# Jiang-Muyun/PointNet12

Hardware: AMD Instinct MI355X
Metric: points/sec fwd+bwd, PointNet2 SemSeg B=16x4096 pts (higher is better)
Workload: dtype f32 (wide-layer products: exact bf16x3 operand splits, 6 bf16 MFMAs per fp32 product, fp32 accumulate)

## Files before the change

### include/pn2.h

```cpp
#ifndef PN2_H
#define PN2_H

#include <stdint.h>

#ifdef __cplusplus
extern "C" {
#endif

#define PN2_ABI_VERSION 15

#define PN2_STAT_REPLICAS 8
#define PN2_DWX_REPLICAS 32

#define PN2_OK 0
#define PN2_OK_SPLIT 1
#define PN2_EINVAL (-1)
#define PN2_ELAUNCH (-2)
#define PN2_EUNSUPPORTED (-3)

typedef void *pn2_stream_t;

typedef struct pn2_bn_lazy {
    const double *stats;
    const float *gamma, *beta;
    float eps, momentum;
    float *running_mean, *running_var;
    int64_t *num_batches_tracked;
    float *affine;
    int64_t count;
    int C;
} pn2_bn_lazy;

typedef struct pn2_bn_coef_lazy {
    const double *red;
    const float *gamma;
    const float *affine;
    float *coef;
    float *dgamma, *dbeta;
    int accumulate;
    int64_t count;
    int C;
} pn2_bn_coef_lazy;

int pn2_version(void);
const char *pn2_error_string(int code);
const char *pn2_last_kernel(void);
void pn2_clear_last_kernel(void);

int pn2_set_option(const char *name, int value);
int pn2_get_option(const char *name, int *value);
const char *pn2_option_name(int index);


int64_t pn2_fps_workspace_bytes(int B, int N, int npoint);
int pn2_fps(const float *xyz, int B, int N, const int64_t *start, int npoint, int64_t *out_idx,
            void *work, pn2_stream_t stream);

int pn2_ball_query(const float *xyz, const float *new_xyz, int B, int N, int S, float r2, int nsample,
                   int64_t *out_idx, pn2_stream_t stream);
int64_t pn2_ball_query_workspace_bytes(int B, int N, int S);
int pn2_ball_query_ws(const float *xyz, const float *new_xyz, int B, int N, int S, float r2, int nsample, int64_t *out_idx,
                      void *work, pn2_stream_t stream);

int pn2_square_distance(const float *src, const float *dst, int B, int S, int N, float *out, pn2_stream_t stream);

// ... 108 lines not shown
int pn2_bwd_res_supported(int64_t P, int C_out, int C_in, int Kpool, int masked);
int pn2_conv1x1_bwd(const float *dZ, int ldz, const float *dZp, int ldo, const int32_t *arg, int Kpool,
                    const float *Y, int ldy, const float *coef, const float *W, int ldw, const float *prev_Y,
                    int ld_prev, const float *prev_affine, float *dXout, int ldxo, double *prev_red, float *dW,
                    int lddw, int64_t P, int C_out, int C_in, const pn2_bn_coef_lazy *coef_lazy, pn2_stream_t stream);

typedef struct {
    const float *W;
    const float *bias;
    int K, N, ldw;
} pn2_eval_layer;
int pn2_fused_eval(const float *X, int ldx, const float *xyz, const float *points, const float *new_xyz,
                   const int64_t *idx, int B, int N, int S, int Knb, int D, int xyz_first,
                   const pn2_eval_layer *layers, int L, int pool, float *out, int ldo, pn2_stream_t stream);

int pn2_invert_index(const int64_t *idx, int B, int M, int T, int32_t *members, int32_t *owners, int32_t *scratch,
                     pn2_stream_t stream);
int pn2_three_interp_bwd_seg(const float *grad_out, int ld, int col0, const int32_t *members, const int32_t *owners,
                             const float *weight, int B, int N, int S, int D, float *grad_points2, pn2_stream_t stream);
int pn2_group_affine_bwd_seg(const float *dZ, int ldz, const float *Y, int ldy, const float *coef, const float *xyz,
                             const float *new_xyz, const int32_t *members, const int32_t *owners, int B, int N, int S,
                             int K, int C, float *G, int ldg, float *dWx, int ldwx, float *dwx_scratch,
                             const pn2_bn_coef_lazy *coef_lazy, pn2_stream_t stream);

int64_t pn2_nll_loss_workspace_bytes(int64_t R);
int pn2_nll_loss_fwd(const float *logp, int ld, const int64_t *target, const float *weight, int64_t R, int C,
                     int64_t ignore_index, void *workspace, float *loss, float *denom, pn2_stream_t stream);
int pn2_nll_loss_bwd(const int64_t *target, const float *weight, int64_t R, int C, int64_t ignore_index,
                     const float *grad_loss, const float *denom, float *dlogp, int ld, pn2_stream_t stream);
int64_t pn2_cross_entropy_workspace_bytes(int64_t R);
int pn2_cross_entropy_fwd(const float *x, int ld, int64_t inner, const int64_t *target, const float *weight, int64_t R, int C,
                          int64_t ignore_index, double label_smoothing, int reduction, void *workspace, float *logsum, float *loss,
                          float *denom, pn2_stream_t stream);
int pn2_cross_entropy_bwd(const float *x, int ld, int64_t inner, const int64_t *target, const float *weight, const float *logsum,
                          int64_t R, int C, int64_t ignore_index, double label_smoothing, int reduction, const float *grad_out,
                          const float *denom, float *dx, pn2_stream_t stream);
int pn2_log_softmax_fwd(const float *x, int ldx, int64_t R, int C, float *out, int ldo, pn2_stream_t stream);
int pn2_log_softmax_bwd(const float *grad_out, int ldg, const float *out, int ldo, int64_t R, int C, float *grad_x, int ldgx,
                        pn2_stream_t stream);

int pn2_adam_step(float *param, float *grad, float *exp_avg, float *exp_avg_sq, int64_t n, double lr, double beta1,
                  double beta2, double eps, double weight_decay, int64_t step, const float *lr_dev, int64_t *step_dev,
                  int zero_grad, pn2_stream_t stream);
int pn2_sgd_step(float *param, float *grad, float *momentum_buf, int64_t n, double lr, double momentum, double dampening,
                 double weight_decay, int nesterov, int maximize, int64_t step, const float *lr_dev, int64_t *step_dev,
                 int zero_grad, pn2_stream_t stream);
// ... 124 lines not shown
```

### pointnet12_amd/_lib.py

```python
import ctypes
import os
import subprocess

_HERE = os.path.dirname(os.path.abspath(__file__))
LIB_PATH = os.environ.get("PN2_LIB_PATH") or os.path.join(_HERE, "libpn2_hip.so")
CSRC = os.path.join(_HERE, "csrc")

_vp, _i, _i64, _f, _d = ctypes.c_void_p, ctypes.c_int, ctypes.c_int64, ctypes.c_float, ctypes.c_double

SIGNATURES = {
    "pn2_version": (_i, []),
    "pn2_error_string": (ctypes.c_char_p, [_i]),
    "pn2_last_kernel": (ctypes.c_char_p, []),
    "pn2_clear_last_kernel": (None, []),
    "pn2_set_option": (_i, [ctypes.c_char_p, _i]),
    "pn2_get_option": (_i, [ctypes.c_char_p, _vp]),
    "pn2_option_name": (ctypes.c_char_p, [_i]),
    "pn2_fps_workspace_bytes": (_i64, [_i, _i, _i]),
    "pn2_fps": (_i, [_vp, _i, _i, _vp, _i, _vp, _vp, _vp]),
    "pn2_ball_query": (_i, [_vp, _vp, _i, _i, _i, _f, _i, _vp, _vp]),
    "pn2_ball_query_workspace_bytes": (_i64, [_i, _i, _i]),
    "pn2_ball_query_ws": (_i, [_vp, _vp, _i, _i, _i, _f, _i, _vp, _vp, _vp]),
    "pn2_square_distance": (_i, [_vp, _vp, _i, _i, _i, _vp, _vp]),
    "pn2_three_nn": (_i, [_vp, _vp, _i, _i, _i, _vp, _vp, _vp, _vp]),
# ... 22 lines not shown
    "pn2_conv1x1_wgrad": (_i, [_vp, _i, _vp, _i, _vp, _i, _vp, _i, _vp, _vp, _i, _vp, _vp, _i, _vp,
                               _i64, _i, _i, _vp, _vp]),
    "pn2_conv1x1_wgrad_workspace_bytes": (_i64, [_i64, _i, _i, _i]),
    "pn2_conv1x1_wgrad_ws": (_i, [_vp, _i, _vp, _i, _vp, _i, _vp, _i, _vp, _vp, _i, _vp, _vp, _i, _vp,
                                  _i64, _i, _i, _vp, _vp, _vp]),
    "pn2_conv1x1_wgrad_cf_scratch_bytes": (_i64, []),
    "pn2_conv1x1_wgrad_cf": (_i, [_vp, _i, _vp, _vp, _i, _vp, _i, _vp, _vp, _vp, _i, _i64, _i, _i, _vp, _vp]),
    "pn2_conv1x1_bwd_pair": (_i, [_vp, _i, _vp, _i, _vp, _i, _vp, _i, _vp, _vp, _i, _vp, _i, _vp, _vp, _i, _vp, _vp, _i, _vp, _vp, _i,
                                  _i64, _i, _i, _vp, _vp]),
    "pn2_res_supported": (_i, [_i64, _i, _i]),
    "pn2_bwd_res_supported": (_i, [_i64, _i, _i, _i, _i]),
    "pn2_conv1x1_bwd": (_i, [_vp, _i, _vp, _i, _vp, _i, _vp, _i, _vp, _vp, _i, _vp, _i, _vp, _vp, _i, _vp, _vp, _i,
                             _i64, _i, _i, _vp, _vp]),
    "pn2_conv1x1_bwd_cf_supported": (_i, [_i64, _i, _i, _i]),
    "pn2_conv1x1_bwd_cf_scratch_bytes": (_i64, [_i, _i]),
    "pn2_conv1x1_bwd_cf": (_i, [_vp, _i, _vp, _i, _vp, _vp, _i, _vp, _vp, _i, _vp, _vp, _i, _vp, _vp, _i, _i64, _i, _i, _vp, _vp, _vp]),
    "pn2_conv1x1_bwd_first_supported": (_i, [_i64, _i, _i, _i]),
    "pn2_conv1x1_bwd_first": (_i, [_vp, _i, _vp, _i, _vp, _vp, _i, _vp, _i, _vp, _vp, _vp, _i, _vp, _i, _i, _vp, _i64, _i, _i, _vp, _vp]),
    "pn2_fused_eval": (_i, [_vp, _i, _vp, _vp, _vp, _vp, _i, _i, _i, _i, _i, _i, _vp, _i, _i, _vp, _i, _vp]),
    "pn2_invert_index": (_i, [_vp, _i, _i, _i, _vp, _vp, _vp, _vp]),
    "pn2_three_interp_bwd_seg": (_i, [_vp, _i, _i, _vp, _vp, _vp, _i, _i, _i, _i, _vp, _vp]),
    "pn2_group_affine_bwd_seg": (_i, [_vp, _i, _vp, _i, _vp, _vp, _vp, _vp, _vp, _i, _i, _i, _i, _i, _vp, _i, _vp, _i,
                                         _vp, _vp, _vp]),
    "pn2_nll_loss_workspace_bytes": (_i64, [_i64]),
    "pn2_nll_loss_fwd": (_i, [_vp, _i, _vp, _vp, _i64, _i, _i64, _vp, _vp, _vp, _vp]),
    "pn2_nll_loss_bwd": (_i, [_vp, _vp, _i64, _i, _i64, _vp, _vp, _vp, _i, _vp]),
    "pn2_cross_entropy_workspace_bytes": (_i64, [_i64]),
    "pn2_cross_entropy_fwd": (_i, [_vp, _i, _i64, _vp, _vp, _i64, _i, _i64, _d, _i, _vp, _vp, _vp, _vp, _vp]),
    "pn2_cross_entropy_bwd": (_i, [_vp, _i, _i64, _vp, _vp, _vp, _i64, _i, _i64, _d, _i, _vp, _vp, _vp, _vp]),
    "pn2_log_softmax_fwd": (_i, [_vp, _i, _i64, _i, _vp, _i, _vp]),
    "pn2_log_softmax_bwd": (_i, [_vp, _i, _vp, _i, _i64, _i, _vp, _i, _vp]),
    "pn2_adam_step": (_i, [_vp, _vp, _vp, _vp, _i64, _d, _d, _d, _d, _d, _i64, _vp, _vp, _i, _vp]),
    "pn2_sgd_step": (_i, [_vp, _vp, _vp, _i64, _d, _d, _d, _d, _i, _i, _i64, _vp, _vp, _i, _vp]),
    "pn2_prepare_clouds": (_i, [_vp, _vp, _vp, _vp, _vp, _vp, _vp, _i, _i, _vp, _vp, _vp, _vp]),
    "pn2_prepare_shapes": (_i, [_vp, _i, _vp, _vp, _vp, _vp, _vp, _i, _vp, _vp, _i, _i, _vp, _vp, _vp, _vp]),
    "pn2_point_transform": (_i, [_vp, _i, _vp, _i, _i, _i, _vp, _i, _vp]),
    "pn2_point_transform_workspace_bytes": (_i64, [_i, _i, _i]),
    "pn2_point_transform_bwd": (_i, [_vp, _i, _vp, _i, _vp, _i, _i, _i, _vp, _i, _vp, _vp, _vp]),
    "pn2_bn_max": (_i, [_vp, _i, _vp, _i64, _i, _i, _vp, _i, _vp, _vp]),
    "pn2_pool_bwd_reduce_noact": (_i, [_vp, _i, _vp, _i, _vp, _i, _vp, _i64, _i, _i, _vp, _vp, _vp]),
    "pn2_conv1x1_fwd_gbias": (_i, [_vp, _i, _vp, _i, _vp, _vp, _i, _i64, _vp, _i, _i64, _i, _i, _vp, _vp]),
    "pn2_group_colsum_workspace_bytes": (_i64, [_i64, _i64, _i]),
    "pn2_group_colsum": (_i, [_vp, _i, _vp, _i, _vp, _i64, _i64, _i, _vp, _i, _vp, _vp]),
    "pn2_conv1x1_fwd_multi": (_i, [_vp, _i, _vp, _i, _vp, _vp, _i, _i64, _vp, _i, _i64, _i, _vp, _vp]),
    "pn2_conv1x1_wgrad_multi": (_i, [_vp, _i, _vp, _i, _vp, _vp, _i, _vp, _i, _vp, _i64, _i, _vp]),
    "pn2_conv1x1_dgrad_multi": (_i, [_vp, _i, _vp, _i, _vp, _vp, _i, _vp, _vp, _vp, _i, _i64, _i, _vp]),
# ... 35 lines not shown
CHANNELS_RGB, CHANNELS_BGR = 0, 1
IMAGE_RGB, IMAGE_HSV = 0, 1
IMAGE_ERR_ROWS = 1
KNN_MAX_K = 32
KNN_ERR_LABEL, KNN_ERR_DST = 1, 2
VOXEL_TILE = 1024
VOXEL_MAX_ROWS = 1 << 29
VOXEL_ERR_RANGE, VOXEL_ERR_ROWS = 1, 2
SEGMENT_MAX_COLS = 16
SEGMENT_ERR_RANGE, SEGMENT_ERR_NONFINITE = 4, 8
CLUSTER_ERR_INDEX, CLUSTER_ERR_CELL, CLUSTER_ERR_CAP, CLUSTER_ERR_ROWS = 16, 32, 64, 128


class BnLazy(ctypes.Structure):
    _fields_ = [("stats", _vp), ("gamma", _vp), ("beta", _vp), ("eps", _f), ("momentum", _f), ("running_mean", _vp),
                ("running_var", _vp), ("num_batches_tracked", _vp), ("affine", _vp), ("count", _i64), ("C", _i)]


class BnCoefLazy(ctypes.Structure):
    _fields_ = [("red", _vp), ("gamma", _vp), ("affine", _vp), ("coef", _vp), ("dgamma", _vp), ("dbeta", _vp),
                ("accumulate", _i), ("count", _i64), ("C", _i)]


class EvalLayer(ctypes.Structure):
    _fields_ = [("W", _vp), ("bias", _vp), ("K", _i), ("N", _i), ("ldw", _i)]


class Src(ctypes.Structure):
    _fields_ = [("X", _vp), ("ldx", _i), ("K", _i), ("affine", _vp), ("relu", _i)]


def src_table(entries):
    return (Src * len(entries))(*[Src(x, ldx, k, aff, relu) for x, ldx, k, aff, relu in entries])


class Pn2Error(RuntimeError):
    pass


def build(force=False):
    if force:
        subprocess.check_call(["make", "-C", CSRC, "-s", "clean"])
    subprocess.check_call(["make", "-C", CSRC, "-s", "-j4"])
    return LIB_PATH


# ... 113 lines not shown
```

### pointnet12_amd/csrc/grouped.hip

```cpp
#include "pn2_common.h"
#include "bn_affine.h"

namespace {

using f32x16 = __attribute__((ext_vector_type(16))) float;

__global__ __launch_bounds__(256) void group_affine_fwd_kernel(const float *__restrict__ Zf, int ldz,
                                                               const float *__restrict__ xyz,
                                                               const float *__restrict__ new_xyz,
                                                               const int64_t *__restrict__ idx,
                                                               const float *__restrict__ Wx, int ldwx, int N, int S,
                                                               int K, int C, int64_t P, float *__restrict__ Y, int ldy,
                                                               double *__restrict__ stats) {
    __shared__ double red[256 * 8];
    const int CG = (C + 3) >> 2;
    const int RPB = 256 / CG;
    const int t = threadIdx.x, cg = t % CG, r = t / CG;
    const bool live = r < RPB;
    const int c = cg * 4;
    float wx[4][3];
#pragma unroll
    for (int e = 0; e < 4; ++e)
#pragma unroll
        for (int a = 0; a < 3; ++a) wx[e][a] = (live && c + e < C) ? Wx[(c + e) * ldwx + a] : 0.f;
    float s0[4] = {0.f, 0.f, 0.f, 0.f}, s1[4] = {0.f, 0.f, 0.f, 0.f};
    double st[8] = {0, 0, 0, 0, 0, 0, 0, 0};
    int since = 0;
    if (live) {
        const int64_t stride = (int64_t)gridDim.x * RPB;
        for (int64_t p0 = (int64_t)blockIdx.x * RPB + r; p0 < P; p0 += 4 * stride) {
            int64_t j[4], g[4], b[4];
#pragma unroll
            for (int u = 0; u < 4; ++u) {
                const int64_t p = p0 + u * stride;
                const bool v = p < P;
                g[u] = v ? p / K : 0;
                b[u] = g[u] / S;
                j[u] = v ? idx[p] : 0;
            }
            float4 z[4];
            float d[4][3];
#pragma unroll
            for (int u = 0; u < 4; ++u) {
                const float *q = xyz + (b[u] * N + j[u]) * 3, *ctr = new_xyz + g[u] * 3;
                d[u][0] = q[0] - ctr[0]; d[u][1] = q[1] - ctr[1]; d[u][2] = q[2] - ctr[2];
                z[u] = *reinterpret_cast<const float4 *>(Zf + (b[u] * N + j[u]) * ldz + c);
            }
#pragma unroll
            for (int u = 0; u < 4; ++u) {
                const int64_t p = p0 + u * stride;
                if (p >= P) break;
                float y[4] = {z[u].x, z[u].y, z[u].z, z[u].w};
#pragma unroll
                for (int e = 0; e < 4; ++e) {
                    y[e] = __builtin_fmaf(wx[e][0], d[u][0], y[e]);
                    y[e] = __builtin_fmaf(wx[e][1], d[u][1], y[e]);
                    y[e] = __builtin_fmaf(wx[e][2], d[u][2], y[e]);
                    if (c + e >= C) y[e] = 0.f;
                    s0[e] += y[e];
                    s1[e] = __builtin_fmaf(y[e], y[e], s1[e]);
                }
                *reinterpret_cast<float4 *>(Y + p * ldy + c) = make_float4(y[0], y[1], y[2], y[3]);
                if (++since == 64) {
#pragma unroll
                    for (int e = 0; e < 4; ++e) {
                        st[e] += (double)s0[e]; st[4 + e] += (double)s1[e];
                        s0[e] = 0.f; s1[e] = 0.f;
                    }
                    since = 0;
                }
            }
        }
#pragma unroll
        for (int e = 0; e < 4; ++e) { st[e] += (double)s0[e]; st[4 + e] += (double)s1[e]; }
    }
    if (stats == nullptr) return;
#pragma unroll
    for (int e = 0; e < 8; ++e) red[t * 8 + e] = st[e];
    __syncthreads();
    for (int ch = t; ch < C; ch += 256) {
        const int g4 = ch >> 2, e = ch & 3;
        double a0 = 0.0, a1 = 0.0;
        for (int rr = 0; rr < RPB; ++rr) {
            a0 += red[(rr * CG + g4) * 8 + e];
            a1 += red[(rr * CG + g4) * 8 + 4 + e];
// ... 244 lines not shown
                       int K, int D, int xyz_first, const float *W, int ldw, const float *bias, float *X, int ldx, float *Y, int ldy,
                       int C_out, double *stats, pn2_stream_t stream) {
    PN2_CHECK_ARG(xyz && W && bias && X && Y && B > 0 && N > 0 && S > 0 && K > 0 && D >= 0 && (D == 0 || points) && (idx || K == N));
    PN2_CHECK_ARG(ldw >= 3 + D && ldx % 4 == 0 && ldx >= ((3 + D + 3) & ~3) && ldy % 4 == 0 && ldy >= C_out);
    const int64_t P = (int64_t)B * S * K;
    if (3 + D > 12 || D > 9 || D < 1 || !idx || !new_xyz || ldx > 12 || !(C_out == 32 || C_out == 64) || P % 64 != 0 || P >= (1LL << 31))
        return PN2_EUNSUPPORTED;
    const int64_t slabs = P / 64;
    int64_t grid = pn2_cdiv(slabs, 4);
    const int64_t cap = (int64_t)pn2_num_cus() * 2;
    if (grid > cap) grid = cap;
    if (C_out == 64)
        hipLaunchKernelGGL(group_conv_fwd_kernel<64>, dim3((unsigned)grid), dim3(256), 0, pn2_s(stream), xyz, points, new_xyz, idx, N, S, K,
                           D, xyz_first, W, ldw, bias, X, ldx, Y, ldy, slabs, stats);
    else
        hipLaunchKernelGGL(group_conv_fwd_kernel<32>, dim3((unsigned)grid), dim3(256), 0, pn2_s(stream), xyz, points, new_xyz, idx, N, S, K,
                           D, xyz_first, W, ldw, bias, X, ldx, Y, ldy, slabs, stats);
    return pn2_launch_status();
}

int pn2_group_affine_fwd(const float *Zf, int ldz, const float *xyz, const float *new_xyz, const int64_t *idx,
                         const float *Wx, int ldwx, int B, int N, int S, int K, int C, float *Y, int ldy, double *stats,
                         pn2_stream_t stream) {
    PN2_CHECK_ARG(Zf && xyz && new_xyz && idx && Wx && Y && B > 0 && N > 0 && S > 0 && K > 0 && C > 0 && C <= 1024 &&
                  ldwx >= 3);
    PN2_CHECK_ARG(ldz % 4 == 0 && ldy % 4 == 0 && ldz >= ((C + 3) & ~3) && ldy >= ((C + 3) & ~3));
    const int64_t P = (int64_t)B * S * K;
    const int rpb = 256 / ((C + 3) >> 2);
    int64_t blocks = pn2_cdiv(P, (int64_t)rpb * 8);
    if (blocks > 1024) blocks = 1024;
    hipLaunchKernelGGL(group_affine_fwd_kernel, dim3((unsigned)blocks), dim3(256), 0, pn2_s(stream), Zf, ldz, xyz, new_xyz, idx,
                       Wx, ldwx, N, S, K, C, P, Y, ldy, stats);
    return pn2_launch_status();
}

int pn2_group_affine_bwd(const float *dZ, int ldz, const float *Y, int ldy, const float *coef, const float *xyz,
                         const float *new_xyz, const int64_t *idx, int B, int N, int S, int K, int C, float *G, int ldg,
                         float *dWx, int ldwx, pn2_stream_t stream) {
    PN2_CHECK_ARG(dZ && Y && coef && xyz && new_xyz && idx && G && dWx && B > 0 && N > 0 && S > 0 && K > 0 && C > 0 &&
                  C <= 1024);
    PN2_CHECK_ARG(ldz % 4 == 0 && ldy % 4 == 0 && ldg % 4 == 0 && ldwx >= 3);
    const int64_t P = (int64_t)B * S * K;
    const int rpb = C < 256 ? 256 / C : 1;
    int64_t blocks = pn2_cdiv(P, (int64_t)rpb * 16);
    if (blocks > 768) blocks = 768;
    hipLaunchKernelGGL(group_affine_bwd_kernel, dim3((unsigned)blocks), dim3(256), 0, pn2_s(stream), dZ, ldz, Y, ldy, coef,
                       (C + 3) & ~3, xyz, new_xyz, idx, N, S, K, C, P, G, ldg, dWx, ldwx);
    return pn2_launch_status();
}
// ... 3 lines not shown
```

### pointnet12_amd/csrc/scatter.hip

```cpp
#include "pn2_common.h"
#include "bn_affine.h"
#include <stdlib.h>

namespace {

__device__ __forceinline__ float4 ld4(const float *p) { return *reinterpret_cast<const float4 *>(p); }

__global__ __launch_bounds__(256) void invert_count_kernel(const int64_t *__restrict__ idx, int M, int T,
                                                           int *__restrict__ counts) {
    const int b = blockIdx.y;
    const int m = blockIdx.x * 256 + threadIdx.x;
    if (m >= M) return;
    const int64_t v = idx[(int64_t)b * M + m];
    if (v >= 0 && v < T) atomicAdd(counts + (int64_t)b * T + v, 1);
}

__global__ __launch_bounds__(1024) void invert_scan_kernel(int *__restrict__ counts, int T, int *__restrict__ offsets) {
    __shared__ int wsum[16];
    __shared__ int carry_s;
    const int b = blockIdx.x, t = threadIdx.x, lane = t & 63, wave = t >> 6;
    int *cnt = counts + (int64_t)b * T;
    int *off = offsets + (int64_t)b * (T + 1);
    if (t == 0) carry_s = 0;
    __syncthreads();
// ... 166 lines not shown
                }
            }
#pragma unroll
            for (int u = 0; u < 4; ++u) {
                if (m[u] < 0) continue;
                if (tg[u] != cur) {
                    if (cur >= 0) {
                        row_flush(grad_points2 + (b * S + cur) * D, c, D, acc, !(first && head_shared));
                        first = false;
                    }
                    acc = make_float4(0.f, 0.f, 0.f, 0.f);
                    cur = tg[u];
                }
                float wu = wt[u];
                PN2_OPAQUE1(wu);
                acc.x = __builtin_fmaf(g[u].x, wu, acc.x); acc.y = __builtin_fmaf(g[u].y, wu, acc.y);
                acc.z = __builtin_fmaf(g[u].z, wu, acc.z); acc.w = __builtin_fmaf(g[u].w, wu, acc.w);
            }
        }
        if (cur >= 0) row_flush(grad_points2 + (b * S + cur) * D, c, D, acc, !(first && head_shared) && cur != tail_next);
    }
}

__global__ __launch_bounds__(256) void group_affine_bwd_seg_kernel(const float *__restrict__ dZ, int ldz,
                                                                   const float *__restrict__ Y, int ldy,
                                                                   const float *coef, int ldc,
                                                                   const float *__restrict__ xyz,
                                                                   const float *__restrict__ new_xyz,
                                                                   const int *__restrict__ members,
                                                                   const int *__restrict__ owners, int N, int S, int K,
                                                                   int C, int lpr_log2, int chunk, int chunks_per_cloud,
                                                                   int64_t chunks, float *__restrict__ G, int ldg,
                                                                   float *__restrict__ dWx, int ldwx,
                                                                   float *__restrict__ rep, LazyCoef lc) {
    __shared__ float red[256 * 12];
    lazy_coef_prologue(lc);
    const int t = threadIdx.x, lane = t & 63;
    const int LPR = 1 << lpr_log2, GPW = 64 >> lpr_log2;
    const int sub = lane & (LPR - 1);
    const int M = S * K;
    const int C4 = (C + 3) & ~3;
    float wacc[4][3];
#pragma unroll
    for (int e = 0; e < 4; ++e) wacc[e][0] = wacc[e][1] = wacc[e][2] = 0.f;
    const int c = sub * 4;
    const bool cv = c < C4;
    float4 c0 = make_float4(0.f, 0.f, 0.f, 0.f), q1 = c0, q0 = c0, mu = c0;
    if (cv) { c0 = ld4(coef + c); q1 = ld4(coef + ldc + c); q0 = ld4(coef + 2 * ldc + c); mu = ld4(coef + 3 * ldc + c); }
    const int64_t qstride = (int64_t)gridDim.x * 4 * GPW;
    for (int64_t q = ((int64_t)blockIdx.x * 4 + (t >> 6)) * GPW + (lane >> lpr_log2); q < chunks; q += qstride) {
        if (!cv) continue;
        const int64_t b = q / chunks_per_cloud;
        const int e0 = (int)(q - b * chunks_per_cloud) * chunk;
        const int e1 = e0 + chunk < M ? e0 + chunk : M;
        const int *mem = members + b * M, *own = owners + b * M;
        const bool head_shared = e0 > 0 && own[e0 - 1] == own[e0];
        const int tail_next = e1 < M ? own[e1] : -1;
        float4 acc = make_float4(0.f, 0.f, 0.f, 0.f);
        int cur = -1;
        bool first = true;
        for (int e = e0; e < e1; e += 4) {
            int m[4], src[4];
            float4 dz[4], y[4];
            float dx[4], dy_[4], dzc[4];
#pragma unroll
            for (int u = 0; u < 4; ++u) {
                const bool v = e + u < e1;
                m[u] = v ? mem[e + u] : -1;
                src[u] = v ? own[e + u] : -1;
            }
#pragma unroll
            for (int u = 0; u < 4; ++u) {
                dz[u] = make_float4(0.f, 0.f, 0.f, 0.f);
                y[u] = mu;
                dx[u] = dy_[u] = dzc[u] = 0.f;
                if (m[u] < 0) continue;
                const int64_t p = b * M + m[u];
                dz[u] = ld4(dZ + p * ldz + c);
                y[u] = ld4(Y + p * ldy + c);
                const float *qp = xyz + (b * N + src[u]) * 3;
                const float *ctr = new_xyz + (b * S + m[u] / K) * 3;
                dx[u] = qp[0] - ctr[0]; dy_[u] = qp[1] - ctr[1]; dzc[u] = qp[2] - ctr[2];
            }
#pragma unroll
            for (int u = 0; u < 4; ++u) {
                if (m[u] < 0) continue;
                if (src[u] != cur) {
                    if (cur >= 0) {
                        row_flush(G + (b * N + cur) * ldg, c, C4, acc, !(first && head_shared));
                        first = false;
                    }
                    acc = make_float4(0.f, 0.f, 0.f, 0.f);
                    cur = src[u];
                }
                float d[4];
                d[0] = __builtin_fmaf(c0.x, dz[u].x, __builtin_fmaf(q1.x, y[u].x - mu.x, q0.x));
                d[1] = __builtin_fmaf(c0.y, dz[u].y, __builtin_fmaf(q1.y, y[u].y - mu.y, q0.y));
                d[2] = __builtin_fmaf(c0.z, dz[u].z, __builtin_fmaf(q1.z, y[u].z - mu.z, q0.z));
                d[3] = __builtin_fmaf(c0.w, dz[u].w, __builtin_fmaf(q1.w, y[u].w - mu.w, q0.w));
                acc.x += d[0]; acc.y += d[1]; acc.z += d[2]; acc.w += d[3];
#pragma unroll
                for (int k = 0; k < 4; ++k) {
                    wacc[k][0] = __builtin_fmaf(d[k], dx[u], wacc[k][0]);
                    wacc[k][1] = __builtin_fmaf(d[k], dy_[u], wacc[k][1]);
                    wacc[k][2] = __builtin_fmaf(d[k], dzc[u], wacc[k][2]);
// ... 56 lines not shown
    pn2_fill_u32(owners, 0xFFFFFFFFu, (int64_t)B * M, s);
    const dim3 grid((unsigned)pn2_cdiv(M, 256), (unsigned)B);
    hipLaunchKernelGGL(invert_count_kernel, grid, dim3(256), 0, s, idx, M, T, counts);
    hipLaunchKernelGGL(invert_scan_kernel, dim3((unsigned)B), dim3(1024), 0, s, counts, T, offsets);
    hipLaunchKernelGGL(invert_fill_kernel, grid, dim3(256), 0, s, idx, M, T, counts, members, owners);
    return pn2_launch_status();
}

int pn2_three_interp_bwd_seg(const float *grad_out, int ld, int col0, const int32_t *members, const int32_t *owners,
                             const float *weight, int B, int N, int S, int D, float *grad_points2, pn2_stream_t stream) {
    PN2_CHECK_ARG(grad_out && members && owners && weight && grad_points2 && B > 0 && N > 0 && S > 0 && D > 0 && col0 >= 0 &&
                  ld >= col0 + D);
    int lpr_log2 = 0;
    while ((4 << lpr_log2) < D && lpr_log2 < 6) ++lpr_log2;
    const int chunk = seg_chunk((int64_t)B * N * 3, 1 << lpr_log2);
    const int cpc = (int)pn2_cdiv((int64_t)N * 3, chunk);
    const int64_t chunks = (int64_t)B * cpc;
    const int64_t waves = pn2_cdiv(chunks, 64 >> lpr_log2);
    hipLaunchKernelGGL(three_interp_bwd_seg_kernel, dim3((unsigned)pn2_cdiv(waves, 4)), dim3(256), 0, pn2_s(stream), grad_out, ld,
                       col0, members, owners, weight, N, S, D, lpr_log2, chunk, cpc, chunks, grad_points2);
    return pn2_launch_status();
}

int pn2_group_affine_bwd_seg(const float *dZ, int ldz, const float *Y, int ldy, const float *coef, const float *xyz,
                             const float *new_xyz, const int32_t *members, const int32_t *owners, int B, int N, int S,
                             int K, int C, float *G, int ldg, float *dWx, int ldwx, float *dwx_scratch,
                             const pn2_bn_coef_lazy *coef_lazy, pn2_stream_t stream) {
    PN2_CHECK_ARG(dZ && Y && coef && xyz && new_xyz && members && owners && G && dWx && B > 0 && N > 0 && S > 0 && K > 0 &&
                  C > 0 && C <= 256 && lazy_coef_ok(coef_lazy, coef, C));
    PN2_CHECK_ARG(ldz % 4 == 0 && ldy % 4 == 0 && ldg % 4 == 0 && ldg >= ((C + 3) & ~3) && ldwx >= 3);
    int lpr_log2 = 0;
    while ((4 << lpr_log2) < C && lpr_log2 < 6) ++lpr_log2;
    const int C4 = (C + 3) & ~3;
    const int chunk = seg_chunk((int64_t)B * S * K, 1 << lpr_log2);
    const int cpc = (int)pn2_cdiv((int64_t)S * K, chunk);
    const int64_t chunks = (int64_t)B * cpc;
    int64_t blocks = pn2_cdiv(pn2_cdiv(chunks, 64 >> lpr_log2), 4);
    if (blocks > 1024) blocks = 1024;
    hipLaunchKernelGGL(group_affine_bwd_seg_kernel, dim3((unsigned)blocks), dim3(256), 0, pn2_s(stream), dZ, ldz, Y, ldy, coef,
                       C4, xyz, new_xyz, members, owners, N, S, K, C, lpr_log2, chunk, cpc, chunks, G, ldg, dWx, ldwx, dwx_scratch,
                       make_lazy_coef(coef_lazy));
    if (dwx_scratch)
        hipLaunchKernelGGL(dwx_fold_kernel, dim3(1), dim3(256), 0, pn2_s(stream), dwx_scratch, C, C4, dWx, ldwx);
    return pn2_launch_status();
}

}
```

### pointnet12_amd/pointnet_util.py

```python
import collections
import contextlib
import ctypes
import types
import weakref
import os

import numpy as np
import torch
import torch.nn as nn

from . import _lib
from ._lib import check as _check, ptr as _p


def timeit(tag, t):
    from time import time
    print("{}: {}s".format(tag, time() - t))
    return time()


def pc_normalize(pc):
    pc = pc - np.mean(pc, axis=0)
    return pc / np.max(np.sqrt(np.sum(pc ** 2, axis=1)))

# ... 491 lines not shown
        g1 = g2 = None
        if D1 and ctx.needs_input_grad[0]:
            g1 = grad_rows.view(B, N, ld)[:, :, :D1]
        if ctx.needs_input_grad[1]:
            g2 = _zeros_f32((B, S, D2), grad_rows.device)
        if ctx.needs_input_grad[1] and inv_off is not None:
            _check(lib.pn2_three_interp_bwd_seg(_p(grad_rows), ld, D1, _p(inv_off), _p(inv_mem), _p(w), B, N, S, D2, _p(g2), st),
                   "pn2_three_interp_bwd_seg")
        elif ctx.needs_input_grad[1]:
            _check(lib.pn2_three_interp_bwd(_p(grad_rows), ld, D1, _p(idx), _p(w), B, N, S, D2, _p(g2), st),
                   "pn2_three_interp_bwd")
        return g1, g2, None, None, None, None



DWX_REPLICAS_SCRATCH = os.environ.get("PN2_DWX_REPLICAS", "1") != "0"
_DIRECT_GRADS = False
LAZY_BN = os.environ.get("PN2_LAZY_BN", "1") == "1"
BWD_PAIR = os.environ.get("PN2_BWD_PAIR_CALL", "1") == "1"
WGRAD_CF = os.environ.get("PN2_WGRAD_CF", "1") != "0"
POOL_IN_EPILOGUE = os.environ.get("PN2_POOL_EPILOGUE", "1") == "1"
GATHER_CONV = os.environ.get("PN2_GATHER_CONV", "1") == "1"
MSG_CONCAT_IN_PLACE = os.environ.get("PN2_MSG_CONCAT_IN_PLACE", "1") == "1"

_REPL = 8
_PAIR_RUNS_SPLIT = set()


def set_direct_grad_accumulation(enabled):
    global _DIRECT_GRADS
    _DIRECT_GRADS = bool(enabled)


def _direct_ok(params):
    if not _DIRECT_GRADS:
        return False
    for q in params:
        g = q.grad
        if g is None or not g.is_contiguous() or g.dtype != torch.float32 or g.device != q.device:
            return False
    return True


def _carve(device, pieces):
    sizes = [n * (torch.finfo(dt).bits // 8) for dt, n in pieces]
    return [v.view(dt) for v, (dt, _) in zip(_zeros_small(sum(sizes), device).split(sizes), pieces)]
# ... 29 lines not shown
    return gathered


def _fwd_factorised(rows, geom, w, b, y, st_l, ci, co, w_pads):
    lib, st = _lib.load(), _lib.stream()
    B, N, D = rows.shape
    S, K = geom.idx.shape[1], geom.idx.shape[2]
    w_ptr = _contig_weight(w).data_ptr()
    wx_ptr, wf_ptr = (w_ptr, w_ptr + 12) if geom.xyz_first else (w_ptr + 4 * D, w_ptr)
    wf_ld = ci
    wf_pad = _padded_feature_columns(w, D, ci, geom.xyz_first)
    if wf_pad is not None:
        w_pads["wf"] = wf_pad
        wf_ptr, wf_ld = wf_pad.data_ptr(), wf_pad.shape[1]
    ldd = _r4(D)
    feat = rows.reshape(B * N, D)
    if ldd != D:
        feat = torch.nn.functional.pad(feat, (0, ldd - D))
    zf = _empty_rows(B * N, co, rows.device)
    _check(lib.pn2_conv1x1_fwd(_p(feat), ldd, None, wf_ptr, wf_ld, _p(b), _p(zf), zf.shape[1], B * N, D, co, None, None, st),
           "pn2_conv1x1_fwd")
    _check(lib.pn2_group_affine_fwd(_p(zf), zf.shape[1], _p(geom.xyz), _p(geom.new_xyz), _p(geom.idx), wx_ptr, ci, B, N, S, K, co,
                                    _p(y), y.shape[1], _p(st_l), st), "pn2_group_affine_fwd")


def _fwd_pooled_last(x, ldx, x_aff, w, b, gamma, y, st_l, ci, co, P, pool, lazy):
    lib, st = _lib.load(), _lib.stream()
    pool_ws = torch.empty(2 * (P // pool) * co, device=x.device, dtype=torch.float32)

    def launch(y):
        return lib.pn2_conv1x1_fwd_pool(_p(x), ldx, _p(x_aff), _p(_contig_weight(w)), ci, _p(b), _p(y), co, P, ci, co, _p(st_l), pool,
                                        _p(gamma), _p(pool_ws), lazy, st)
    rc = launch(y)
    if rc == _lib.PN2_EUNSUPPORTED and y is None:
        y = _empty_rows(P, co, x.device)
        rc = launch(y)
    if rc != _lib.PN2_EUNSUPPORTED:
        _check(rc, "pn2_conv1x1_fwd_pool")
        return y, pool_ws
    _check(lib.pn2_conv1x1_fwd(_p(x), ldx, _p(x_aff), _p(_contig_weight(w)), ci, _p(b), _p(y), y.shape[1], P, ci, co, _p(st_l), lazy, st),
           "pn2_conv1x1_fwd")
    return y, None


def _fwd_plain(x, ldx, x_aff, w, b, y, st_l, ci, co, P, lazy, w_pads, l):
    w_rd, w_ld = _aligned_weight(w, ci, co, P)
# ... 92 lines not shown
                                        _p(s.flat[7 * a.l + 1]), _p(scratch), _p(a.dW), a.ci, s.P, a.co, a.ci, coef_lazy, st),
               "pn2_conv1x1_wgrad_cf")
        return dx, a.dW, None
    ws_bytes = lib.pn2_conv1x1_wgrad_workspace_bytes(s.P, a.co, a.ci, int(a.pooled)) if s.training else 0
    if ws_bytes:
        ws = torch.empty(ws_bytes, device=s.dev, dtype=torch.uint8)
        _check(lib.pn2_conv1x1_wgrad_ws(*dy, _p(a.x), a.ldx, _p(a.x_aff), _p(a.dW), a.ci, None, s.P, a.co, a.ci, coef_lazy, _p(ws), st),
               "pn2_conv1x1_wgrad_ws")
    else:
        _check(lib.pn2_conv1x1_wgrad(*dy, _p(a.x), a.ldx, _p(a.x_aff), _p(a.dW), a.ci, None if s.training else _p(a.dbias), s.P, a.co,
                                     a.ci, coef_lazy, st), "pn2_conv1x1_wgrad")
    return dx, a.dW, None


def _first_layer_bwd(s, a):
    lib, st, geom, feats, dZ, y, co, dev = s.lib, s.st, s.ctx.geom, s.rows, a.dZ, a.y, a.co, s.dev
    B, N, D = feats.shape
    S, K = geom.idx.shape[1], geom.idx.shape[2]
    ldc, ldd = _r4(co), _r4(D)
    dW = s.flat[0].grad if s.direct else _zeros_f32((co, 3 + D), dev)
    ldw = 3 + D
    x_col, f_col = (0, 3) if geom.xyz_first else (D, 0)
    G = _zeros_f32((B * N, ldc), dev)
    if geom.inv is not None and co <= 256:
        scratch = _zeros_small(4 * _lib.DWX_REPLICAS * 3 * ldc, dev) if DWX_REPLICAS_SCRATCH else None
        _check(lib.pn2_group_affine_bwd_seg(_p(dZ), dZ.shape[1], _p(y), y.shape[1], _p(a.coef), _p(geom.xyz), _p(geom.new_xyz),
                                            _p(geom.inv[0]), _p(geom.inv[1]), B, N, S, K, co, _p(G), ldc,
                                            dW.data_ptr() + 4 * x_col, ldw, _p(scratch), a.coef_lazy, st), "pn2_group_affine_bwd_seg")
    else:
        _check(lib.pn2_group_affine_bwd(_p(dZ), dZ.shape[1], _p(y), y.shape[1], _p(a.coef), _p(geom.xyz), _p(geom.new_xyz),
                                        _p(geom.idx), B, N, S, K, co, _p(G), ldc, dW.data_ptr() + 4 * x_col, ldw, st),
               "pn2_group_affine_bwd")
    feat = feats.reshape(B * N, D)
    if ldd != D:
        feat = torch.nn.functional.pad(feat, (0, ldd - D)).contiguous()
    dy = _UpGrad.linear(G, co)
    _check(lib.pn2_conv1x1_wgrad(*dy, _p(feat), ldd, None, dW.data_ptr() + 4 * f_col, ldw, None, B * N, co, D, None, st),
           "pn2_conv1x1_wgrad")
    d_feats = None
    if s.ctx.needs_input_grad[0]:
        wf_ptr = _contig_weight(a.w).data_ptr() + (12 if geom.xyz_first else 0)
        wf_ld = 3 + D
        if "wf" in s.ctx.w_pads:
            wf_ptr, wf_ld = s.ctx.w_pads["wf"].data_ptr(), s.ctx.w_pads["wf"].shape[1]
        dF = _empty_rows(B * N, D, dev)
        _check(lib.pn2_conv1x1_dgrad(*dy, wf_ptr, wf_ld, None, 0, None, _p(dF), ldd, None, B * N, co, D, None, st), "pn2_conv1x1_dgrad")
        d_feats = (dF[:, :D] if ldd != D else dF).reshape(B, N, D)
    return d_feats, dW, None


class _SharedMLP(torch.autograd.Function):

    @staticmethod
    def forward(ctx, rows, c_in, pool, training, bn_cfg, geom, dest, *flat):
        lib, st = _lib.load(), _lib.stream()
        dev = rows.device
        L = len(flat) // 7
        P = rows.shape[0] if geom is None else rows.shape[0] * geom.idx.shape[1] * geom.idx.shape[2]
        chans = [c_in] + [flat[7 * l].shape[0] for l in range(L)]
        pieces = _carve(dev, ([(torch.float64, _REPL * 2 * c) for c in chans[1:]] if training else []) +
                        [(torch.float32, 4 * _r4(c)) for c in chans[1:]])
        stats, affs = pieces[:-L] or [None] * L, pieces[-L:]
        Ys = []
        x, ldx, x_aff = rows, rows.shape[-1], None
        pool_ws = gathered = None
        w_pads = {}
        lazy_on = training and LAZY_BN
        lazy_prev = None
        keep = []
        for l in range(L):
            w, b, gamma, beta, rmean, rvar, nbt = flat[7 * l:7 * l + 7]
            co, ci = chans[l + 1], chans[l]
            st_l, aff = stats[l], affs[l]
            lazy = None if lazy_prev is None else ctypes.byref(lazy_prev)
            pooled_last = (l == L - 1 and pool and training and x_aff is not None and POOL_IN_EPILOGUE and P % 32 == 0 and
                           (pool == 16 or pool % 32 == 0) and co % 32 == 0)
            no_y = bool(pooled_last and lazy_on and lib.pn2_conv1x1_bwd_cf_supported(P, co, ci, pool))
            y = None if no_y else _empty_rows(P, co, dev)
            if l == 0 and geom is not None and geom.gather:
                gathered = _fwd_gather_conv(rows, geom, w, b, y, st_l, ci, co, P)
            elif l == 0 and geom is not None:
                _fwd_factorised(rows, geom, w, b, y, st_l, ci, co, w_pads)
            elif pooled_last:
                y, pool_ws = _fwd_pooled_last(x, ldx, x_aff, w, b, gamma, y, st_l, ci, co, P, pool, lazy)
            else:
                _fwd_plain(x, ldx, x_aff, w, b, y, st_l, ci, co, P, lazy, w_pads, l)
            lazy_prev = None
            eps, mom = bn_cfg[l]
            if lazy_on:
                lazy_prev = _lib.BnLazy(_p(st_l), _p(gamma), _p(beta), eps, mom, _p(rmean), _p(rvar), _p(nbt), _p(aff), P, co)
                keep.append(lazy_prev)
            else:
                _check(lib.pn2_bn_finalize(_p(st_l), P, co, _p(gamma), _p(beta), eps, mom, int(training),
                                           _p(rmean), _p(rvar), _p(nbt), _p(aff), st), "pn2_bn_finalize")
            Ys.append(y)
            x, ldx, x_aff = y, (y.shape[1] if y is not None else 0), aff
        lazy = None if lazy_prev is None else ctypes.byref(lazy_prev)
        cl = chans[-1]
        K = pool if pool else 1
        G = P // K
        if dest is not None and pool and cl % 4 == 0:
            big, col0 = dest
            out = big[:, col0:col0 + cl]
        else:
            out = _empty_rows(G, cl, dev)
        ldo = out.stride(0)
        arg = torch.empty(G, ldo, device=dev, dtype=torch.int32) if pool else None
        if pool_ws is not None:
            _check(lib.pn2_bn_pool_select(_p(pool_ws), _p(affs[-1]), G, cl, _p(out), ldo, _p(arg), lazy, st), "pn2_bn_pool_select")
        else:
            _check(lib.pn2_bn_relu_max(_p(Ys[-1]), Ys[-1].shape[1], _p(affs[-1]), G, K, cl, _p(out), ldo, _p(arg), lazy, st),
                   "pn2_bn_relu_max")
        if training:
            bump_param_generation()
        ctx.meta = (chans, pool, bool(training), P)
        ctx.geom = geom
        ctx.gather = tuple(rows.shape) if gathered is not None else None
        if gathered is not None:
            rows = gathered
        ctx.params = flat
        ctx.w_pads = w_pads
        ctx.save_for_backward(rows, out, arg, *Ys, *affs, *[flat[7 * l] for l in range(L)],
                              *[flat[7 * l + 2] for l in range(L)], pool_ws if Ys[-1] is None else None)
        return out[:, :cl] if out.shape[1] != cl else out

    @staticmethod
    def backward(ctx, grad_out):
        lib, st = _lib.load(), _lib.stream()
        chans, pool, training, P = ctx.meta
        saved = ctx.saved_tensors
        L = len(chans) - 1
        rows, out, arg = saved[:3]
        Ys, affs, Ws, gammas = (saved[3 + i * L:3 + (i + 1) * L] for i in range(4))
        dev, flat = rows.device, ctx.params
        cl = chans[-1]
        ldo = out.stride(0)
        ld_grad = ldo
        if pool and grad_out.dim() == 2 and grad_out.stride(1) == 1 and grad_out.stride(0) >= cl and grad_out.dtype == torch.float32:
            ld_grad = grad_out.stride(0)
        else:
            if ldo != cl:
                g = torch.zeros(out.shape[0], ldo, device=dev, dtype=torch.float32)
                g[:, :cl] = grad_out
                grad_out = g
# ... 501 lines not shown
```

Baseline: 13.40 million.

## Recompute first-layer grouped activations in backward from per-point features instead of reading Y

Adds a gather variant of the segmented group-affine backward kernel. It rebuilds the pre-BN output of the first factorised layer from the per-point projected features Zf, the xyz offsets and the Wx weights, instead of loading the stored grouped tensor Y. The forward path returns Zf and keeps it on ctx for backward. It also prefetches member/owner indices one step ahead. Y is still allocated and written in forward, so the intent is to cut backward read traffic on a large B*S*K tensor. The cost is a gather and a few FMAs per element, plus keeping Zf alive until backward.

New measurement: 13.46 million (median of 6 runs). About the same (+0.5%).

```diff
diff --git a/include/pn2.h b/include/pn2.h
--- a/include/pn2.h
+++ b/include/pn2.h
@@ -41,6 +41,15 @@
     int64_t count;
     int C;
 } pn2_bn_coef_lazy;
+
+typedef struct pn2_affine_gather {
+    const float *Zf; int ldz;
+    const float *xyz;
+    const float *new_xyz;
+    const int64_t *idx;
+    const float *Wx; int ldwx;
+    int B, N, S, K, C;
+} pn2_affine_gather;
 
 int pn2_version(void);
 const char *pn2_error_string(int code);
@@ -195,6 +204,9 @@
                              const float *new_xyz, const int32_t *members, const int32_t *owners, int B, int N, int S,
                              int K, int C, float *G, int ldg, float *dWx, int ldwx, float *dwx_scratch,
                              const pn2_bn_coef_lazy *coef_lazy, pn2_stream_t stream);
+int pn2_group_affine_bwd_seg_gather(const float *dZ, int ldz, const pn2_affine_gather *src, const float *coef,
+                                    const int32_t *members, const int32_t *owners, float *G, int ldg, float *dWx, int ldwx,
+                                    float *dwx_scratch, const pn2_bn_coef_lazy *coef_lazy, pn2_stream_t stream);
 
 int64_t pn2_nll_loss_workspace_bytes(int64_t R);
 int pn2_nll_loss_fwd(const float *logp, int ld, const int64_t *target, const float *weight, int64_t R, int C,
diff --git a/pointnet12_amd/_lib.py b/pointnet12_amd/_lib.py
--- a/pointnet12_amd/_lib.py
+++ b/pointnet12_amd/_lib.py
@@ -68,6 +68,7 @@
     "pn2_three_interp_bwd_seg": (_i, [_vp, _i, _i, _vp, _vp, _vp, _i, _i, _i, _i, _vp, _vp]),
     "pn2_group_affine_bwd_seg": (_i, [_vp, _i, _vp, _i, _vp, _vp, _vp, _vp, _vp, _i, _i, _i, _i, _i, _vp, _i, _vp, _i,
                                          _vp, _vp, _vp]),
+    "pn2_group_affine_bwd_seg_gather": (_i, [_vp, _i, _vp, _vp, _vp, _vp, _vp, _i, _vp, _i, _vp, _vp, _vp]),
     "pn2_nll_loss_workspace_bytes": (_i64, [_i64]),
     "pn2_nll_loss_fwd": (_i, [_vp, _i, _vp, _vp, _i64, _i, _i64, _vp, _vp, _vp, _vp]),
     "pn2_nll_loss_bwd": (_i, [_vp, _vp, _i64, _i, _i64, _vp, _vp, _vp, _i, _vp]),
@@ -149,6 +150,11 @@
                 ("accumulate", _i), ("count", _i64), ("C", _i)]
 
 
+class AffineGather(ctypes.Structure):
+    _fields_ = [("Zf", _vp), ("ldz", _i), ("xyz", _vp), ("new_xyz", _vp), ("idx", _vp), ("Wx", _vp), ("ldwx", _i),
+                ("B", _i), ("N", _i), ("S", _i), ("K", _i), ("C", _i)]
+
+
 class EvalLayer(ctypes.Structure):
     _fields_ = [("W", _vp), ("bias", _vp), ("K", _i), ("N", _i), ("ldw", _i)]
 
diff --git a/pointnet12_amd/csrc/affine_gather.h b/pointnet12_amd/csrc/affine_gather.h
--- /dev/null
+++ b/pointnet12_amd/csrc/affine_gather.h
@@ -0,0 +1,54 @@
+#pragma once
+#include "pn2_common.h"
+
+struct AffineGather {
+    const float *Zf; int ldz;
+    const float *xyz, *new_xyz;
+    const int64_t *idx;
+    const float *Wx; int ldwx;
+    int N, S, K;
+};
+
+namespace {
+
+struct AffineGatherRow { float4 z; float d[3]; };
+
+__device__ __forceinline__ void affine_gather_wx(const float *Wx, int ldwx, int c, int C, bool live, float (&wx)[4][3]) {
+#pragma unroll
+    for (int e = 0; e < 4; ++e)
+#pragma unroll
+        for (int a = 0; a < 3; ++a) wx[e][a] = (live && c + e < C) ? Wx[(c + e) * ldwx + a] : 0.f;
+}
+
+__device__ __forceinline__ void affine_gather_request(const float *Zf, int ldz, const float *xyz, const float *new_xyz, int64_t src,
+                                                      int64_t grp, int c, AffineGatherRow &r) {
+    const float *q = xyz + src * 3, *ctr = new_xyz + grp * 3;
+    r.d[0] = q[0] - ctr[0]; r.d[1] = q[1] - ctr[1]; r.d[2] = q[2] - ctr[2];
+    r.z = *reinterpret_cast<const float4 *>(Zf + src * ldz + c);
+}
+
+__device__ __forceinline__ float4 affine_gather_finish(const AffineGatherRow &r, const float (&wx)[4][3]) {
+    float y[4] = {r.z.x, r.z.y, r.z.z, r.z.w};
+    float d0 = r.d[0], d1 = r.d[1], d2 = r.d[2];
+    PN2_OPAQUE3(d0, d1, d2);
+#pragma unroll
+    for (int e = 0; e < 4; ++e) {
+        y[e] = __builtin_fmaf(wx[e][0], d0, y[e]);
+        y[e] = __builtin_fmaf(wx[e][1], d1, y[e]);
+        y[e] = __builtin_fmaf(wx[e][2], d2, y[e]);
+    }
+    return make_float4(y[0], y[1], y[2], y[3]);
+}
+
+static inline AffineGather make_affine_gather(const pn2_affine_gather *a) {
+    AffineGather o{};
+    if (a && a->Zf) o = AffineGather{a->Zf, a->ldz, a->xyz, a->new_xyz, a->idx, a->Wx, a->ldwx, a->N, a->S, a->K};
+    return o;
+}
+
+static inline bool affine_gather_ok(const pn2_affine_gather *a, int C) {
+    return a && a->Zf && a->xyz && a->new_xyz && a->Wx && a->B > 0 && a->N > 0 && a->S > 0 && a->K > 0 && a->C == C &&
+           a->ldz % 4 == 0 && a->ldz >= ((C + 3) & ~3) && a->ldwx >= 3 && (reinterpret_cast<uintptr_t>(a->Zf) & 15) == 0;
+}
+
+}
diff --git a/pointnet12_amd/csrc/grouped.hip b/pointnet12_amd/csrc/grouped.hip
--- a/pointnet12_amd/csrc/grouped.hip
+++ b/pointnet12_amd/csrc/grouped.hip
@@ -1,5 +1,6 @@
 #include "pn2_common.h"
 #include "bn_affine.h"
+#include "affine_gather.h"
 
 namespace {
 
@@ -19,10 +20,7 @@
     const bool live = r < RPB;
     const int c = cg * 4;
     float wx[4][3];
-#pragma unroll
-    for (int e = 0; e < 4; ++e)
-#pragma unroll
-        for (int a = 0; a < 3; ++a) wx[e][a] = (live && c + e < C) ? Wx[(c + e) * ldwx + a] : 0.f;
+    affine_gather_wx(Wx, ldwx, c, C, live, wx);
     float s0[4] = {0.f, 0.f, 0.f, 0.f}, s1[4] = {0.f, 0.f, 0.f, 0.f};
     double st[8] = {0, 0, 0, 0, 0, 0, 0, 0};
     int since = 0;
@@ -38,29 +36,22 @@
                 b[u] = g[u] / S;
                 j[u] = v ? idx[p] : 0;
             }
-            float4 z[4];
-            float d[4][3];
-#pragma unroll
-            for (int u = 0; u < 4; ++u) {
-                const float *q = xyz + (b[u] * N + j[u]) * 3, *ctr = new_xyz + g[u] * 3;
-                d[u][0] = q[0] - ctr[0]; d[u][1] = q[1] - ctr[1]; d[u][2] = q[2] - ctr[2];
-                z[u] = *reinterpret_cast<const float4 *>(Zf + (b[u] * N + j[u]) * ldz + c);
-            }
+            AffineGatherRow row[4];
+#pragma unroll
+            for (int u = 0; u < 4; ++u) affine_gather_request(Zf, ldz, xyz, new_xyz, b[u] * N + j[u], g[u], c, row[u]);
 #pragma unroll
             for (int u = 0; u < 4; ++u) {
                 const int64_t p = p0 + u * stride;
                 if (p >= P) break;
-                float y[4] = {z[u].x, z[u].y, z[u].z, z[u].w};
+                const float4 yq = affine_gather_finish(row[u], wx);
+                float y[4] = {yq.x, yq.y, yq.z, yq.w};
 #pragma unroll
                 for (int e = 0; e < 4; ++e) {
-                    y[e] = __builtin_fmaf(wx[e][0], d[u][0], y[e]);
-                    y[e] = __builtin_fmaf(wx[e][1], d[u][1], y[e]);
-                    y[e] = __builtin_fmaf(wx[e][2], d[u][2], y[e]);
                     if (c + e >= C) y[e] = 0.f;
                     s0[e] += y[e];
                     s1[e] = __builtin_fmaf(y[e], y[e], s1[e]);
                 }
-                *reinterpret_cast<float4 *>(Y + p * ldy + c) = make_float4(y[0], y[1], y[2], y[3]);
+                if (Y != nullptr) *reinterpret_cast<float4 *>(Y + p * ldy + c) = make_float4(y[0], y[1], y[2], y[3]);
                 if (++since == 64) {
 #pragma unroll
                     for (int e = 0; e < 4; ++e) {
@@ -351,9 +342,9 @@
 int pn2_group_affine_fwd(const float *Zf, int ldz, const float *xyz, const float *new_xyz, const int64_t *idx,
                          const float *Wx, int ldwx, int B, int N, int S, int K, int C, float *Y, int ldy, double *stats,
                          pn2_stream_t stream) {
-    PN2_CHECK_ARG(Zf && xyz && new_xyz && idx && Wx && Y && B > 0 && N > 0 && S > 0 && K > 0 && C > 0 && C <= 1024 &&
+    PN2_CHECK_ARG(Zf && xyz && new_xyz && idx && Wx && (Y || stats) && B > 0 && N > 0 && S > 0 && K > 0 && C > 0 && C <= 1024 &&
                   ldwx >= 3);
-    PN2_CHECK_ARG(ldz % 4 == 0 && ldy % 4 == 0 && ldz >= ((C + 3) & ~3) && ldy >= ((C + 3) & ~3));
+    PN2_CHECK_ARG(ldz % 4 == 0 && ldz >= ((C + 3) & ~3) && (Y == nullptr || (ldy % 4 == 0 && ldy >= ((C + 3) & ~3))));
     const int64_t P = (int64_t)B * S * K;
     const int rpb = 256 / ((C + 3) >> 2);
     int64_t blocks = pn2_cdiv(P, (int64_t)rpb * 8);
diff --git a/pointnet12_amd/csrc/scatter.hip b/pointnet12_amd/csrc/scatter.hip
--- a/pointnet12_amd/csrc/scatter.hip
+++ b/pointnet12_amd/csrc/scatter.hip
@@ -1,5 +1,6 @@
 #include "pn2_common.h"
 #include "bn_affine.h"
+#include "affine_gather.h"
 #include <stdlib.h>
 
 namespace {
@@ -212,8 +213,9 @@
     }
 }
 
+template <bool GATHER>
 __global__ __launch_bounds__(256) void group_affine_bwd_seg_kernel(const float *__restrict__ dZ, int ldz,
-                                                                   const float *__restrict__ Y, int ldy,
+                                                                   const float *__restrict__ Y, int ldy, const AffineGather ag,
                                                                    const float *coef, int ldc,
                                                                    const float *__restrict__ xyz,
                                                                    const float *__restrict__ new_xyz,
@@ -237,6 +239,8 @@
     const bool cv = c < C4;
     float4 c0 = make_float4(0.f, 0.f, 0.f, 0.f), q1 = c0, q0 = c0, mu = c0;
     if (cv) { c0 = ld4(coef + c); q1 = ld4(coef + ldc + c); q0 = ld4(coef + 2 * ldc + c); mu = ld4(coef + 3 * ldc + c); }
+    float wx[4][3];
+    if (GATHER) affine_gather_wx(ag.Wx, ag.ldwx, c, C, cv, wx);
     const int64_t qstride = (int64_t)gridDim.x * 4 * GPW;
     for (int64_t q = ((int64_t)blockIdx.x * 4 + (t >> 6)) * GPW + (lane >> lpr_log2); q < chunks; q += qstride) {
         if (!cv) continue;
@@ -249,28 +253,43 @@
         float4 acc = make_float4(0.f, 0.f, 0.f, 0.f);
         int cur = -1;
         bool first = true;
+        int mn[4], srcn[4];
+        auto request_members = [&](int e) {
+#pragma unroll
+            for (int u = 0; u < 4; ++u) {
+                const int eu = e + u < e1 ? e + u : e1 - 1;
+                const int mv = mem[eu], sv = own[eu];
+                mn[u] = e + u < e1 ? mv : -1;
+                srcn[u] = e + u < e1 ? sv : -1;
+            }
+        };
+        request_members(e0);
         for (int e = e0; e < e1; e += 4) {
             int m[4], src[4];
             float4 dz[4], y[4];
             float dx[4], dy_[4], dzc[4];
 #pragma unroll
-            for (int u = 0; u < 4; ++u) {
-                const bool v = e + u < e1;
-                m[u] = v ? mem[e + u] : -1;
-                src[u] = v ? own[e + u] : -1;
-            }
-#pragma unroll
-            for (int u = 0; u < 4; ++u) {
-                dz[u] = make_float4(0.f, 0.f, 0.f, 0.f);
-                y[u] = mu;
-                dx[u] = dy_[u] = dzc[u] = 0.f;
-                if (m[u] < 0) continue;
-                const int64_t p = b * M + m[u];
+            for (int u = 0; u < 4; ++u) { m[u] = mn[u]; src[u] = srcn[u]; }
+            request_members(e + 4 < e1 ? e + 4 : e);
+#pragma unroll
+            for (int u = 0; u < 4; ++u) {
+                const int mc = m[u] < 0 ? 0 : m[u], sc = m[u] < 0 ? 0 : src[u];
+                const int64_t p = b * M + mc;
                 dz[u] = ld4(dZ + p * ldz + c);
-                y[u] = ld4(Y + p * ldy + c);
-                const float *qp = xyz + (b * N + src[u]) * 3;
-                const float *ctr = new_xyz + (b * S + m[u] / K) * 3;
-                dx[u] = qp[0] - ctr[0]; dy_[u] = qp[1] - ctr[1]; dzc[u] = qp[2] - ctr[2];
+                if (GATHER) {
+                    AffineGatherRow row;
+                    affine_gather_request(ag.Zf, ag.ldz, xyz, new_xyz, b * N + sc, b * S + mc / K, c, row);
+                    dx[u] = row.d[0]; dy_[u] = row.d[1]; dzc[u] = row.d[2];
+                    y[u] = affine_gather_finish(row, wx);
+                    if (c + 1 >= C) y[u].y = 0.f;
+                    if (c + 2 >= C) y[u].z = 0.f;
+                    if (c + 3 >= C) y[u].w = 0.f;
+                } else {
+                    y[u] = ld4(Y + p * ldy + c);
+                    const float *qp = xyz + (b * N + sc) * 3;
+                    const float *ctr = new_xyz + (b * S + mc / K) * 3;
+                    dx[u] = qp[0] - ctr[0]; dy_[u] = qp[1] - ctr[1]; dzc[u] = qp[2] - ctr[2];
+                }
             }
 #pragma unroll
             for (int u = 0; u < 4; ++u) {
@@ -373,11 +392,11 @@
     return pn2_launch_status();
 }
 
-int pn2_group_affine_bwd_seg(const float *dZ, int ldz, const float *Y, int ldy, const float *coef, const float *xyz,
-                             const float *new_xyz, const int32_t *members, const int32_t *owners, int B, int N, int S,
-                             int K, int C, float *G, int ldg, float *dWx, int ldwx, float *dwx_scratch,
-                             const pn2_bn_coef_lazy *coef_lazy, pn2_stream_t stream) {
-    PN2_CHECK_ARG(dZ && Y && coef && xyz && new_xyz && members && owners && G && dWx && B > 0 && N > 0 && S > 0 && K > 0 &&
+static int launch_affine_bwd_seg(const float *dZ, int ldz, const float *Y, int ldy, const AffineGather &ag, const float *coef,
+                                 const float *xyz, const float *new_xyz, const int32_t *members, const int32_t *owners, int B,
+                                 int N, int S, int K, int C, float *G, int ldg, float *dWx, int ldwx, float *dwx_scratch,
+                                 const pn2_bn_coef_lazy *coef_lazy, pn2_stream_t stream) {
+    PN2_CHECK_ARG(dZ && coef && xyz && new_xyz && members && owners && G && dWx && B > 0 && N > 0 && S > 0 && K > 0 &&
                   C > 0 && C <= 256 && lazy_coef_ok(coef_lazy, coef, C));
     PN2_CHECK_ARG(ldz % 4 == 0 && ldy % 4 == 0 && ldg % 4 == 0 && ldg >= ((C + 3) & ~3) && ldwx >= 3);
     int lpr_log2 = 0;
@@ -388,7 +407,8 @@
     const int64_t chunks = (int64_t)B * cpc;
     int64_t blocks = pn2_cdiv(pn2_cdiv(chunks, 64 >> lpr_log2), 4);
     if (blocks > 1024) blocks = 1024;
-    hipLaunchKernelGGL(group_affine_bwd_seg_kernel, dim3((unsigned)blocks), dim3(256), 0, pn2_s(stream), dZ, ldz, Y, ldy, coef,
+    auto kern = ag.Zf ? group_affine_bwd_seg_kernel<true> : group_affine_bwd_seg_kernel<false>;
+    hipLaunchKernelGGL(kern, dim3((unsigned)blocks), dim3(256), 0, pn2_s(stream), dZ, ldz, Y, ldy, ag, coef,
                        C4, xyz, new_xyz, members, owners, N, S, K, C, lpr_log2, chunk, cpc, chunks, G, ldg, dWx, ldwx, dwx_scratch,
                        make_lazy_coef(coef_lazy));
     if (dwx_scratch)
@@ -396,4 +416,21 @@
     return pn2_launch_status();
 }
 
-}
+int pn2_group_affine_bwd_seg(const float *dZ, int ldz, const float *Y, int ldy, const float *coef, const float *xyz,
+                             const float *new_xyz, const int32_t *members, const int32_t *owners, int B, int N, int S,
+                             int K, int C, float *G, int ldg, float *dWx, int ldwx, float *dwx_scratch,
+                             const pn2_bn_coef_lazy *coef_lazy, pn2_stream_t stream) {
+    PN2_CHECK_ARG(Y);
+    return launch_affine_bwd_seg(dZ, ldz, Y, ldy, AffineGather{}, coef, xyz, new_xyz, members, owners, B, N, S, K, C, G, ldg, dWx, ldwx,
+                                 dwx_scratch, coef_lazy, stream);
+}
+
+int pn2_group_affine_bwd_seg_gather(const float *dZ, int ldz, const pn2_affine_gather *src, const float *coef,
+                                    const int32_t *members, const int32_t *owners, float *G, int ldg, float *dWx, int ldwx,
+                                    float *dwx_scratch, const pn2_bn_coef_lazy *coef_lazy, pn2_stream_t stream) {
+    PN2_CHECK_ARG(src && affine_gather_ok(src, src->C));
+    return launch_affine_bwd_seg(dZ, ldz, nullptr, 0, make_affine_gather(src), coef, src->xyz, src->new_xyz, members, owners, src->B,
+                                 src->N, src->S, src->K, src->C, G, ldg, dWx, ldwx, dwx_scratch, coef_lazy, stream);
+}
+
+}
diff --git a/pointnet12_amd/pointnet_util.py b/pointnet12_amd/pointnet_util.py
--- a/pointnet12_amd/pointnet_util.py
+++ b/pointnet12_amd/pointnet_util.py
@@ -537,6 +537,7 @@
 POOL_IN_EPILOGUE = os.environ.get("PN2_POOL_EPILOGUE", "1") == "1"
 GATHER_CONV = os.environ.get("PN2_GATHER_CONV", "1") == "1"
 MSG_CONCAT_IN_PLACE = os.environ.get("PN2_MSG_CONCAT_IN_PLACE", "1") == "1"
+AFFINE_GATHER = int(os.environ.get("PN2_AFFINE_GATHER", "1"))
 
 _REPL = 8
 _PAIR_RUNS_SPLIT = set()
@@ -612,6 +613,7 @@
            "pn2_conv1x1_fwd")
     _check(lib.pn2_group_affine_fwd(_p(zf), zf.shape[1], _p(geom.xyz), _p(geom.new_xyz), _p(geom.idx), wx_ptr, ci, B, N, S, K, co,
                                     _p(y), y.shape[1], _p(st_l), st), "pn2_group_affine_fwd")
+    return zf if AFFINE_GATHER >= 1 and geom.inv is not None and co <= 256 else None
 
 
 def _fwd_pooled_last(x, ldx, x_aff, w, b, gamma, y, st_l, ci, co, P, pool, lazy):
@@ -750,7 +752,16 @@
     ldw = 3 + D
     x_col, f_col = (0, 3) if geom.xyz_first else (D, 0)
     G = _zeros_f32((B * N, ldc), dev)
-    if geom.inv is not None and co <= 256:
+    zf = s.ctx.affine_zf
+    if zf is not None:
+        scratch = _zeros_small(4 * _lib.DWX_REPLICAS * 3 * ldc, dev) if DWX_REPLICAS_SCRATCH else None
+        w_ptr = _contig_weight(a.w).data_ptr()
+        src = _lib.AffineGather(_p(zf), zf.shape[1], _p(geom.xyz), _p(geom.new_xyz), _p(geom.idx), w_ptr + 4 * x_col, 3 + D,
+                                B, N, S, K, co)
+        _check(lib.pn2_group_affine_bwd_seg_gather(_p(dZ), dZ.shape[1], ctypes.byref(src), _p(a.coef), _p(geom.inv[0]), _p(geom.inv[1]),
+                                                   _p(G), ldc, dW.data_ptr() + 4 * x_col, ldw, _p(scratch), a.coef_lazy, st),
+               "pn2_group_affine_bwd_seg_gather")
+    elif geom.inv is not None and co <= 256:
         scratch = _zeros_small(4 * _lib.DWX_REPLICAS * 3 * ldc, dev) if DWX_REPLICAS_SCRATCH else None
         _check(lib.pn2_group_affine_bwd_seg(_p(dZ), dZ.shape[1], _p(y), y.shape[1], _p(a.coef), _p(geom.xyz), _p(geom.new_xyz),
                                             _p(geom.inv[0]), _p(geom.inv[1]), B, N, S, K, co, _p(G), ldc,
@@ -791,7 +802,7 @@
         stats, affs = pieces[:-L] or [None] * L, pieces[-L:]
         Ys = []
         x, ldx, x_aff = rows, rows.shape[-1], None
-        pool_ws = gathered = None
+        pool_ws = gathered = affine_zf = None
         w_pads = {}
         lazy_on = training and LAZY_BN
         lazy_prev = None
@@ -808,7 +819,7 @@
             if l == 0 and geom is not None and geom.gather:
                 gathered = _fwd_gather_conv(rows, geom, w, b, y, st_l, ci, co, P)
             elif l == 0 and geom is not None:
-                _fwd_factorised(rows, geom, w, b, y, st_l, ci, co, w_pads)
+                affine_zf = _fwd_factorised(rows, geom, w, b, y, st_l, ci, co, w_pads)
             elif pooled_last:
                 y, pool_ws = _fwd_pooled_last(x, ldx, x_aff, w, b, gamma, y, st_l, ci, co, P, pool, lazy)
             else:
@@ -848,6 +859,7 @@
             rows = gathered
         ctx.params = flat
         ctx.w_pads = w_pads
+        ctx.affine_zf = affine_zf
         ctx.save_for_backward(rows, out, arg, *Ys, *affs, *[flat[7 * l] for l in range(L)],
                               *[flat[7 * l + 2] for l in range(L)], pool_ws if Ys[-1] is None else None)
         return out[:, :cl] if out.shape[1] != cl else out
```
